# mike-gimelfarb/bboptpy

Hardware: AMD Instinct MI355X
Metric: candidate-evals/sec (higher is better)
Workload: dtype f64; 1 GPU; ActiveCMAES n=128 np=4096 rosenbrock, 256 independent populations per GPU in lockstep; populations_per_gpu=256, n=128, np=4096, objective=rosenbrock

## Files before the change

bboptpy_amd/csrc/bbo_cma.hip:

```cpp
#include "bbo_cma_kernels.hpp"
#include "bbo_sep_kernels.hpp"
#include "bbo_chol_kernels.hpp"
#include "bbo_eig_mw.hpp"

#include <algorithm>
#include <atomic>
#include <cmath>
#include <cstdlib>
#include <limits>

namespace bbo {

namespace {

enum { K_SAMPLE = 0, K_RANK, K_WHITEN, K_GRAM, K_PATHS, K_COV, K_EIGEN, K_POST, K_STOP, K_COUNT };
static const char *const K_NAMES[K_COUNT] = { "bbo:cma_sample_eval", "bbo:cma_rank", "bbo:cma_whiten", "bbo:cma_gram", "bbo:cma_paths", "bbo:cma_cov", "bbo:cma_eigen", "bbo:cma_post", "bbo:cma_history_stop" };

int pick_maxt(int ld)
{
    const int per_wave = ((ld >> 4) + 3) / 4;
    if (per_wave <= 1) return 1;
    if (per_wave <= 2) return 2;
    if (per_wave <= 4) return 4;
    return 8;
// ... 310 lines not shown
            C_.upload(cm.data(), P * ld2);
        } else {
            B_.alloc(P * ld2);
            C_.alloc(P * ld2);
            B_.upload(eye.data(), P * ld2);
            C_.upload(eye.data(), P * ld2);
        }
        isc_.upload(eye.data(), P * ld2);
    }
    D_.upload(ones.data(), P * ld);
    keep_bc_ = dense;
    last_n_ = n;

    std::vector<double> xm(P * ld, 0.);
    for (int p = 0; p < P; p++) std::copy(guess + (size_t) p * n, guess + (size_t) (p + 1) * n,
            xm.begin() + p * ld);
    xmean_.upload(xm.data(), P * ld);

    std::vector<CmaScal> sc(P);
    for (auto &s : sc) {
        std::memset(&s, 0, sizeof(s));
        s.sigma = params_.sigma0;
        s.fbest = -std::numeric_limits<double>::infinity();
        s.fworst = std::numeric_limits<double>::infinity();
        s.hist_head = -1;
        s.basis_ok = same_shape ? 0 : 1;
    }
    scal_.upload(sc.data(), P);
    basis_maybe_stale_ = same_shape;

    if (dense) eig_work_.alloc((size_t) P * 4 * eig_slab((int) ld));

    CmaDev &d = d_;
    d = CmaDev {};
    d.X = X_.p; d.f = f_.p; d.rank = rank_.p; d.order = order_.p;
    d.xmean = xmean_.p; d.xold = xold_.p; d.pc = pc_.p; d.ps = ps_.p;
    d.C = C_.p; d.B = B_.p; d.D = D_.p; d.isc = isc_.p; d.BDp = BDp_.p; d.ISp = ISp_.p;
    d.A = chol ? A_.p : nullptr;
    d.chol_repairs = chol ? chol_repairs_.p : nullptr;
    d.S = S_.p; d.zn2 = zn2_.p; d.csep = csep_.p; d.gram_part = gram_part_.p; d.mean_part = mean_part_.p;
    d.hist_best = hist_best_.p; d.hist_kth = hist_kth_.p; d.eig_work = eig_work_.p;
    d.weights = weights_.p; d.lower = lower_.p; d.upper = upper_.p; d.aux = aux_.p;
    d.zinject = nullptr; d.zrecord = nullptr; d.scal = scal_.p;
    d.stamps = stamps_.p;
    d.mw_fail_host = mw_fail_host_;
    d.mw_fault = mw_fault_from_env();
    mw_release();

    if (obj_.is_program()) {
        prog_.bind(obj_.program, params_.device, n, P);
        std::vector<ProgPlan> plan(P);
        for (int p = 0; p < P; p++)
            plan[p] = ProgPlan { X_.p + (size_t) p * c.lambda_pad * ld, f_.p + (size_t) p * c.lambda_pad, lambda,
                    c.ld };
        prog_.upload_plan(plan);
        std::vector<double> finf((size_t) P * c.lambda_pad, std::numeric_limits<double>::infinity());
        f_.upload(finf.data(), finf.size());
    } else
        prog_.unbind();

    c.honor_stop = 0;
    inited_ = true;
    if (dense) {
        launch_post(2);
        BBO_HIP(hipGetLastError());
        BBO_HIP(hipStreamSynchronize(stream_));
    }
}

void CmaEngine::launch_post(int mode)
{
    const CmaConst &c = c_;
    if (c.ld <= 128) {
        const size_t lds = (size_t) (c.ld * (c.ld + 2) + c.ld) * sizeof(double);
        allow_lds((const void*) cma_post_mfma<1>, 140 * 1024);
        allow_lds((const void*) cma_post_mfma<4>, 140 * 1024);
        if (c.npop < 32)
            hipLaunchKernelGGL(cma_post_mfma<4>, dim3(c.npop, 4), dim3(256), lds, stream_, d_, c_,
                    mode);
        else
            hipLaunchKernelGGL(cma_post_mfma<1>, dim3(c.npop, 1), dim3(256), lds, stream_, d_, c_,
                    mode);
    } else {
        dim3 grid(c.ld / 16, c.ld / 16, c.npop);
        hipLaunchKernelGGL(cma_post, grid, dim3(256), 0, stream_, d_, c_, mode);
    }
}

SampleRoute CmaEngine::sample_route() const
{
    const CmaConst &c = c_;
    SampleRoute r {};
    r.gy = c.npop;
    r.writes_zn = c.variant != 2;
    auto is = [&r](SampleKernel k, int gx, int block, size_t lds) {
        r.k = k;
        r.gx = gx;
        r.block = block;
        r.lds = lds;
    };
    if (c.variant == 2) {
        const int per_pop = std::max(1, 4096 / c.npop);
        if (c.ld <= 256)
            is(SK_SEP_16, std::min((c.lambda_pad + 15) / 16, per_pop), 256, (size_t) 16 * c.ld * sizeof(double));
        else if (c.ld <= 2048) {
            is(SK_SEP_64_512, std::min((c.lambda_pad + 7) / 8, per_pop), 512, (size_t) 8 * c.ld * sizeof(double));
            r.full = nothing_to_guard() ? 1 : 0;
            if (r.full && sep_sum_objective(c.obj) && !(d_.dbg & DBG_SEP_ROWS_LDS))
                is(c.ld == 1024 && c.obj != OBJ_RASTRIGIN && c.obj != OBJ_DIFFPOW ? SK_SEP_SUM4 : SK_SEP_SUM,
                        std::min(c.lambda_pad / (4 * SEP_K), per_pop), 256, 0);
            else if (r.full)
                r.k = SK_SEP_64_512_LEAN;
        } else
            is(SK_SEP_64, std::min((c.lambda_pad + 3) / 4, per_pop), 256, (size_t) 4 * c.ld * sizeof(double));
    } else if (c.ld == 128 && (long) c.npop * c.lambda_pad >= sample128_min_rows_
            && (c.obj < 0 || frag_objective_ok(c.obj))) {
        r.rows_per_wg = rows_per_workgroup((long) c.npop * c.lambda_pad, 4096);
        is(c.variant == 3 && chol_tri_ ? SK_EVAL128_TRI : SK_EVAL128, (c.lambda_pad + r.rows_per_wg - 1) / r.rows_per_wg,
                512, 128 * 1024);
        r.full = nothing_to_guard() ? 1 : 0;
    } else if (c.ld == 128 && (long) c.npop * (c.lambda_pad / 16) <= sample_wide_max_tiles_)
        is(c.variant == 3 && chol_tri_ ? SK_TILE8_TRI : SK_TILE8, c.lambda_pad / 16, 512,
                (size_t) 16 * (c.ld + 2) * sizeof(double));
    else if (c.ld <= 128)
        is(c.ld <= 32 ? SK_EVAL64_1_8 : c.ld <= 64 ? SK_EVAL64_1 : SK_EVAL64_2, (c.lambda_pad + 63) / 64, 256,
                (size_t) 64 * (c.ld + 2) * sizeof(double));
    else {
        const int tiles = c.lambda_pad / 16;
        const size_t lds = (size_t) 16 * (c.ld + 2) * sizeof(double);
        if ((long) tiles * c.npop <= 32 && c.ld <= 256 && !(d_.dbg & DBG_SAMPLE_4WAVES))
            is(SK_TILE16, tiles, 1024, lds);
        else
            is(pick_maxt(c.ld) == 4 ? SK_EVAL_4 : SK_EVAL_8, tiles, 256, lds);
    }
    return r;
}

void CmaEngine::launch_sample_eval()
{
    const SampleRoute r = sample_route();
    auto go = [&](auto kernel, int allow, auto... args) {
        if (allow) allow_lds((const void*) kernel, allow);
        hipLaunchKernelGGL(kernel, dim3(r.gx, r.gy), dim3(r.block), r.lds, stream_, d_, c_, args...);
    };
    timer_.begin(stream_, K_SAMPLE);
    switch (r.k) {
    case SK_NONE: break;
    case SK_SEP_16: go(sep_sample_eval<16>, 128 * 1024); break;
    case SK_SEP_64_512: go(sep_sample_eval<64, 512>, 140 * 1024); break;
    case SK_SEP_64_512_LEAN: go(sep_sample_eval<64, 512, true>, 140 * 1024); break;
    case SK_SEP_SUM: go(sep_sum_kernel<0>(c_.obj), 0); break;
    case SK_SEP_SUM4: go(sep_sum_kernel<4>(c_.obj), 0); break;
    case SK_SEP_64: go(sep_sample_eval<64>, 140 * 1024); break;
    case SK_EVAL128: go(cma_sample_eval128, 128 * 1024, r.rows_per_wg, r.full); break;
    case SK_EVAL128_TRI: go(cma_sample_eval128_tri, 128 * 1024, r.rows_per_wg, r.full); break;
    case SK_TILE8: go(cma_sample_eval<1, 8>, 0); break;
    case SK_TILE8_TRI: go(cma_sample_eval<1, 8, true>, 0); break;
    case SK_EVAL64_1_8: go(cma_sample_eval64<1, 8>, 0); break;
    case SK_EVAL64_1: go(cma_sample_eval64<1>, 80 * 1024); break;
    case SK_EVAL64_2: go(cma_sample_eval64<2>, 80 * 1024); break;
    case SK_TILE16: go(cma_sample_eval<1, 16>, 0); break;
    case SK_EVAL_4: go(cma_sample_eval<4>, 0); break;
    case SK_EVAL_8: go(cma_sample_eval<8>, 80 * 1024); break;
    }
    timer_.end(stream_);
    BBO_HIP(hipGetLastError());
    c_.use_zn = (r.writes_zn && !c_.bound) ? 1 : 0;
    last_sample_ = r;
}

void CmaEngine::launch_rank()
{
    const CmaConst &c = c_;
    rank_wrote_norms_ = false;
    timer_.begin(stream_, K_RANK);
    last_rank_ = rank_route(c.lambda, c.npop, d_.dbg);
    switch (last_rank_) {
    case RK_WAVE:
        hipLaunchKernelGGL(cma_rank_wave, dim3((c.npop + 3) / 4), dim3(256), 0, stream_, d_, c_);
        break;
    case RK_COUNT64:
        hipLaunchKernelGGL(cma_rank64, dim3((c.lambda + 3) / 4, c.npop), dim3(256), 0, stream_, d_, c_);
        break;
    case RK_COUNT32:
        hipLaunchKernelGGL(cma_rank32, dim3((c.lambda + 7) / 8, c.npop), dim3(256), 0, stream_, d_, c_);
        break;
    case RK_COUNT8:
        hipLaunchKernelGGL(cma_rank, dim3((c.lambda + 31) / 32, c.npop), dim3(256), 0, stream_, d_, c_);
        break;
    default: {
        const int m = rank_sort_m(c.lambda);
        allow_lds((const void*) cma_rank_sort, 128 * 1024);
        const size_t lds = rank_sort_merges(m, d_.dbg) ? (size_t) m * 24 : (size_t) std::max(m, 1024) * 12;
        hipLaunchKernelGGL(cma_rank_sort, dim3(c.npop), dim3(sort_threads(m)), lds, stream_, d_,
                c_, m);
        break;
    }
    }
    if (last_rank_ != RK_WAVE) rank_wrote_norms_ = c.variant == 1 && c.use_zn && !basis_maybe_stale_;
    timer_.end(stream_);
    BBO_HIP(hipGetLastError());
}

UpdateRoute CmaEngine::update_route(bool norms_done, bool with_cov) const
{
    const CmaConst &c = c_;
    UpdateRoute r {};
    auto add = [&r](UpdateKernel k, int slot, int gx, int gy, int gz, int block, size_t lds = 0, int arg = 0) {
        r.step[r.count++] = UpdateRoute::Step { k, slot, gx, gy, gz, block, lds, arg };
    };
    const int NT = c.ld / 16, LT = NT * (NT + 1) / 2;
    if (c.variant == 3) {
        const int in_lds = c.ld <= 128 ? 1 : 0;
        add(UK_CHOL_PATHS, K_PATHS, c.npop, 1, 1, 256);
        add(UK_CHOL_CPRIME, K_GRAM, LT, c.npop, 1, 256);
        add(UK_CHOL_FACTOR, K_COV, c.npop, 1, 1, 256, in_lds ? (size_t) c.ld * (c.ld + 1) * sizeof(double) : 0, in_lds);
        return r;
    }
    if (c.variant == 2) {
        add(UK_SEP_MOMENTS, K_GRAM, c.splits, (c.ld + 511) / 512, c.npop, 256);
        add(UK_SEP_PATHS, K_PATHS, c.npop, 1, 1, 256);
        return r;
    }
    if (c.variant == 1 && !norms_done) {
        if (c.ld == 128 && (long) c.npop * c.mu_pad >= 256 * 128) {
            const int rw = rows_per_workgroup((long) c.npop * c.mu_pad, 2048);
            add(UK_WHITEN128, K_WHITEN, (c.mu_pad + rw - 1) / rw, c.npop, 1, 512, (size_t) (128 * 128 + 128) * sizeof(double),
                    rw);
        } else
            add(UK_WHITEN, K_WHITEN, c.mu_pad / 16, c.npop, 1, 256, (size_t) (16 * (c.ld + 2) + 64) * sizeof(double),
                    pick_maxt(c.ld));
    }
    if (c.ld != 128)
        add(UK_GRAM, K_GRAM, c.splits, (LT + 4 * GRAM_TPW - 1) / (4 * GRAM_TPW), c.npop, 256, gram_lds_bytes(c.ld, c.rps),
                gram_ldy(c.ld));
    else if (d_.dbg & DBG_GRAM128_LDS)
        add(UK_GRAM128, K_GRAM, c.splits, c.npop, 1, 256, (size_t) (2 * G128_CH * G128_LDY + 4 * G128_CH) * sizeof(double));
    else
        add(UK_GRAM128S, K_GRAM, c.splits, c.npop, 1, 256);
    if (c.lazy_isc && c.n >= 64 && !(d_.dbg & DBG_PATHS_LAZY256))
        add(UK_PATHS_LAZY1K, K_PATHS, c.npop, 1, 1, 1024);
    else
        add(c.lazy_isc ? UK_PATHS_LAZY : UK_PATHS, K_PATHS, c.npop, 1, 1, 256);
    if (with_cov) add(UK_COV, K_COV, (c.n * (c.n + 1) / 2 + 255) / 256, c.npop, 1, 256);
    return r;
}

static auto whiten_kernel(int maxt) -> void (*)(CmaDev, CmaConst)
{
    switch (maxt) {
    case 1: return cma_whiten<1>;
    case 2: return cma_whiten<2>;
    case 4: return cma_whiten<4>;
    default: return cma_whiten<8>;
    }
}

void CmaEngine::launch_update(bool with_cov)
{
    const bool norms_done = rank_wrote_norms_;
    rank_wrote_norms_ = false;
    const UpdateRoute r = update_route(norms_done, with_cov);
    for (int i = 0; i < r.count; i++) {
        const UpdateRoute::Step &s = r.step[i];
        auto go = [&](auto kernel, int allow, auto... args) {
            if (allow) allow_lds((const void*) kernel, allow);
            hipLaunchKernelGGL(kernel, dim3(s.gx, s.gy, s.gz), dim3(s.block), s.lds, stream_, d_, c_, args...);
        };
        timer_.begin(stream_, s.slot);
        switch (s.k) {
        case UK_CHOL_PATHS: go(chol_paths, 0); break;
        case UK_CHOL_CPRIME: go(chol_cprime, 0); break;
        case UK_CHOL_FACTOR: go(chol_factor, 0, s.arg); break;
        case UK_SEP_MOMENTS: go(sep_moments, 0); break;
        case UK_SEP_PATHS: go(sep_paths, 0); break;
        case UK_WHITEN128: go(cma_whiten128, 132 * 1024, s.arg); break;
        case UK_WHITEN: go(whiten_kernel(s.arg), s.arg == 8 ? 80 * 1024 : 0); break;
        case UK_GRAM128S: go(cma_gram128s, 0); break;
        case UK_GRAM128: go(cma_gram128, 80 * 1024); break;
        case UK_GRAM: go(cma_gram, (int) GRAM_LDS_MAX, s.arg); break;
        case UK_PATHS: go(cma_paths, 0); break;
        case UK_PATHS_LAZY: go(cma_paths_lazy, 0); break;
        case UK_PATHS_LAZY1K: go(cma_paths_lazy1k, 0); break;
        case UK_COV: go(cma_cov, 0); break;
        }
        timer_.end(stream_);
        BBO_HIP(hipGetLastError());
    }
    last_update_ = r;
}

int CmaEngine::next_mw_xcd()
{
    static std::atomic<int> counter { 0 };
    return counter.fetch_add(1) & 7;
}

EigRoute CmaEngine::eig_route(bool spread_ok, bool fuse_ok) const
{
    const CmaConst &c = c_;
    const int dbg = d_.dbg;
    EigRoute r {};
    if (c.variant >= 2) return r;
    auto add = [&r](EigKernel k, int arg = 0) { r.step[r.count++] = EigRoute::Step { k, arg }; };
    const EigPlan pl_lds = eig_plan(c.n, c.ld);
    r.split = pl_lds.use_lds && pl_lds.threads == 512 && pl_lds.dc && c.npop <= split_maxp_
            && !(dbg & (DBG_QL | DBG_DC_NO_MERGES | DBG_DC_NO_LEAVES | DBG_TRED_L2 | DBG_EIG_ONE_WG));
    const EigPlan pl = r.split ? eig_plan_split(c.n, c.ld) : pl_lds;
// ... 259 lines not shown
        launch_eigen(eig_route());
        BBO_HIP(hipStreamSynchronize(stream_));
    }
    timer_.collect();
    prog_timer_.collect();
}

void CmaEngine::inject_normals(const double *z, int count)
{
    BBO_REQUIRE(inited_, "inject_normals before init");
    rank_wrote_norms_ = false;
    if (!z) {
        d_.zinject = nullptr;
        return;
    }
    const size_t want = (size_t) c_.npop * c_.lambda * c_.n;
    BBO_REQUIRE((size_t) count == want, "inject_normals: count must be populations*lambda*n");
    if (zinject_.count != want) zinject_.alloc(want);
    zinject_.upload(z, want);
    d_.zinject = zinject_.p;
}

void CmaEngine::after_chunk(bool in_run)
{
    if (in_run) return;
    if (mw_check_failed()) {
        launch_eigen(eig_route());
        BBO_HIP(hipStreamSynchronize(stream_));
    }
}

void CmaEngine::inspect(const std::vector<CmaScal> &sc)
{
    bool stale = false;
    for (const auto &s : sc) stale = stale || !s.basis_ok;
    basis_maybe_stale_ = stale;
    mw_check_failed();
    for (const auto &s : sc)
        if (s.eig_mw_fail && !mw_disabled_) {
            mw_disabled_ = true;
            mw_release();
        }
}

int CmaEngine::chunk_limit(int want)
{
    return small_fused_ok() ? std::min(want, 512) : want;
}

void CmaEngine::launch_chunk(int gens)
{
    if (small_fused_ok()) launch_small(gens, true);
    else Engine::launch_chunk(gens);
}

void CmaEngine::solution(int population, double *x_out, int *n_evals, int *converged)
{
    enter_population("solution()", population);
    CmaScal s;
    scal_.download(&s, 1, population);
    std::vector<double> x(c_.ld);
    if (s.it <= 0) xmean_.download(x.data(), c_.ld, (size_t) population * c_.ld);
    else X_.download(x.data(), c_.ld, ((size_t) population * c_.lambda_pad + s.ibw[0]) * c_.ld);
    std::copy(x.begin(), x.begin() + c_.n, x_out);
    *n_evals = s.fev;
    if (s.it <= 0) {
        *converged = c_.variant == 3 ? (c_.tol >= 0. ? 1 : 0) : (0 >= c_.mit) ? 1 : 0;
    } else {
        *converged = s.flag != 0 ? 1 : 0;
    }
}

void CmaEngine::optimize(int n, const double *lower, const double *upper, const double *guess,
        const ObjectiveSpec &obj, double *x_out, int *n_evals, int *converged)
{
    init(n, lower, upper, guess, obj);
    const int max_gen = c_.mfev / c_.lambda + 2;
    run(max_gen);
    CmaScal s;
    scal_.download(&s, 1, 0);
    std::vector<double> x(c_.ld);
    if (s.it <= 0) xmean_.download(x.data(), c_.ld, 0);
    else X_.download(x.data(), c_.ld, (size_t) s.ibw[0] * c_.ld);
    std::copy(x.begin(), x.begin() + c_.n, x_out);
    *n_evals = s.fev;
    *converged = (s.stop == 1) ? 1 : 0;
}

double CmaEngine::evaluate_point(const double *x)
{
    if (obj_.needs_host()) {
        double f = 0.;
        obj_.eval_host(x, 1, c_.n, c_.n, &f);
        return f;
    }
    if (obj_.is_program()) {
        BBO_HIP(hipSetDevice(params_.device));
        return prog_.evaluate_point(stream_, x);
    }
    return builtin_objective_host(obj_.builtin, c_.n, x, aux_h_.data());
}

int CmaEngine::get(const std::string &k, int p, double *out, int cap)
{
    enter_population("get()", p);
    const CmaConst &c = c_;
    const size_t ld = c.ld, n = c.n;
    const StateOut o { out, cap };
    if (c.variant == 2 && (k == "B" || k == "C" || k == "invsqrtC" || k == "ycoeff"))
        throw Error(BBO_ERR_KEY, "SepCMAES keeps a diagonal covariance: read 'csep' and 'D'");
    if (c.variant == 3 && (k == "B" || k == "C" || k == "D" || k == "invsqrtC" || k == "ycoeff" || k == "csep"))
        throw Error(BBO_ERR_KEY, "CholeskyCMAES keeps the factor: read 'A'");
    if (k == "A") {
        if (c.variant != 3) throw Error(BBO_ERR_KEY, "'A' belongs to CholeskyCMAES");
        return o.rows(A_, p * ld, c.n, c.n, c.ld);
    }
    if (k == "xmean") return o.vec(xmean_, p * ld, (int) n);
    if (k == "xold") return o.vec(xold_, p * ld, (int) n);
    if (k == "pc") return o.vec(pc_, p * ld, (int) n);
    if (k == "ps") return o.vec(ps_, p * ld, (int) n);
    if (k == "D") return o.vec(D_, p * ld, (int) n);
    if (k == "csep") return o.vec(csep_, p * ld, (int) n);
    if (k == "B") return o.rows(B_, p * ld, c.n, c.n, c.ld);
    if (k == "C") return o.rows(C_, p * ld, c.n, c.n, c.ld);
    if (k == "invsqrtC") {
        if (c.lazy_isc && out) {
            const int hs = c_.honor_stop;
            c_.honor_stop = 0;
            launch_post(3);
            c_.honor_stop = hs;
            BBO_HIP(hipGetLastError());
            BBO_HIP(hipStreamSynchronize(stream_));
        }
        return o.rows(isc_, p * ld, c.n, c.n, c.ld);
    }
    if (k == "BD") {
        if (out && cap >= (int) (n * n)) {
            std::vector<double> pk(ld * ld);
            BDp_.download(pk.data(), ld * ld, p * ld * ld);
            for (size_t i = 0; i < n; i++)
                for (size_t j = 0; j < n; j++) out[i * n + j] = pk[bfrag_index(i, j, ld)];
        }
        return (int) (n * n);
    }
    if (k == "arx") return o.rows(X_, (size_t) p * c.lambda_pad, c.lambda, c.n, c.ld);
    if (k == "weights") {
        if (out && cap >= c.mu) weights_.download(out, c.mu);
        return c.mu;
    }
    if (k == "fitness") {
        if (out && cap >= c.lambda) f_.download(out, c.lambda, (size_t) p * c.lambda_pad);
        return c.lambda;
    }
    if (k == "fit_idx" || k == "fit_val" || k == "rank") {
        if (out && cap >= c.lambda) {
            std::vector<int> ord(c.lambda);
            (k == "rank" ? rank_ : order_).download(ord.data(), c.lambda,
                    (size_t) p * c.lambda_pad);
            if (k == "fit_val") {
                std::vector<double> f(c.lambda);
                f_.download(f.data(), c.lambda, (size_t) p * c.lambda_pad);
                for (int i = 0; i < c.lambda; i++) out[i] = f[ord[i]];
            } else {
                for (int i = 0; i < c.lambda; i++) out[i] = ord[i];
            }
        }
        return c.lambda;
    }
    if (k == "ycoeff") {
        if (out && cap >= c.mu) {
            std::vector<double> S(c.mu_pad);
            S_.download(S.data(), c.mu_pad, (size_t) p * c.mu_pad);
            for (int i = 0; i < c.mu; i++) out[i] = S[i] / std::max(S[c.mu - 1 - i], 1e-8);
        }
        return c.mu;
    }
    if (k == "zlast") {
        const size_t cnt = (size_t) c.lambda * n;
        if (!zrecord_.p) return 0;
        if (out && cap >= (int) cnt) zrecord_.download(out, cnt, p * cnt);
        return (int) cnt;
    }
    if (k == "profile") return profile_report(out, cap);
    if (const int r = prog_get(k, out, cap); r >= 0) return r;
    if (k == "eig_work") {
        const size_t cnt = std::min((size_t) 4 * eig_slab(c.ld), eig_work_.count);
        if (out && (size_t) cap >= cnt) eig_work_.download(out, cnt, (size_t) p * 4 * eig_slab(c.ld));
        return (int) cnt;
    }
    if (k == "eig_stamps") {
        if (!stamps_.p) return 0;
        if (out && cap >= 48) {
            long long t[48];
            stamps_.download(t, 48);
            for (int i = 0; i < 48; i++) out[i] = (double) t[i];
        }
        return 48;
    }
    if (k == "best_hist" || k == "kth_hist") {
        if (out && cap >= c.hlen)
            (k == "best_hist" ? hist_best_ : hist_kth_).download(out, c.hlen, (size_t) p * c.hlen);
        return c.hlen;
    }
    CmaScal s;
    scal_.download(&s, 1, p);
    if (k == "sigma") return o.one(s.sigma);
    if (k == "it") return o.one(s.it);
    if (k == "fev") return o.one(s.fev);
    if (k == "flag") return o.one(s.flag);
    if (k == "stop") return o.one(s.stop);
    if (k == "hsig") return o.one(s.hsig);
    if (k == "pslen") return o.one(s.pslen);
    if (k == "fbest") return o.one(s.fbest);
    if (k == "fworst") return o.one(s.fworst);
    if (k == "eigenlastev") return o.one(s.eigenlastev);
    if (k == "eigen_done") return o.one(s.eigen_done);
    if (k == "basis_ok") return o.one(s.basis_ok);
    if (k == "eig_stage") return o.one(s.eig_stage);
    if (k == "eig_mw_fail") return o.one(s.eig_mw_fail);
    if (k == "chol_repairs") {
        if (c.variant != 3) throw Error(BBO_ERR_KEY, "'chol_repairs' belongs to CholeskyCMAES");
        int r = 0;
        chol_repairs_.download(&r, 1, p);
        return o.one(r);
    }
    if (c.variant == 3 && k == "chol_tri") return o.one(chol_tri_ ? 1 : 0);
    if (c.variant == 3 && k == "stol") return o.one(c.stol);
    if (c.variant == 3 && k == "ranked") return o.one(c.ranked);
    if (k == "eig_mw_off") return o.one(mw_disabled_ ? 1 : 0);
    if (k == "eig_split_maxp") return o.one(split_maxp_);
    if (k == "eig_fixed128") return o.one(last_route_.fixed ? 1 : 0);
    if (k == "cov_fused") return o.one(last_route_.forms_c ? 1 : 0);
    if (k == "eig_route") {
        double ids[sizeof(last_route_.step) / sizeof(last_route_.step[0])];
        for (int i = 0; i < last_route_.count; i++) ids[i] = last_route_.step[i].k;
        return o.copy(ids, last_route_.count);
    }
    if (k == "rank_route") return o.one(last_rank_);
    if (k == "sample_route") return o.one(last_sample_.k);
    if (k == "sample_lean") return o.one(last_sample_.full);
    if (k == "update_route") {
        double ids[sizeof(last_update_.step) / sizeof(last_update_.step[0])];
        for (int i = 0; i < last_update_.count; i++) ids[i] = last_update_.step[i].k;
        return o.copy(ids, last_update_.count);
    }
    if (k == "small_fused") return o.one(small_fused_ ? 1 : 0);
    if (k == "splits") return o.one(c.splits);
    if (k == "eig_mw_reserved") return o.one((double) mw_reserved_);
    if (k == "eig_mw_capacity") {
        MwBudget &b = MwBudget::get();
        std::lock_guard<std::mutex> lock(b.m);
        return o.one((double) b.capacity(params_.device));
    }
    if (k == "best_len") return o.one(s.hist_len);
    if (k == "best_buffer") return o.one(s.hist_head);
    if (k == "ibest") return o.one(s.ibw[0]);
    if (k == "ybw") return o.copy(s.ybw, 4);
    if (k == "ibw") {
        const double ids[4] = { (double) s.ibw[0], (double) s.ibw[1], (double) s.ibw[2], (double) s.ibw[3] };
        return o.copy(ids, 4);
    }
    if (k == "n") return o.one(c.n);
    if (k == "lambda") return o.one(c.lambda);
    if (k == "mu") return o.one(c.mu);
    if (k == "mueff") return o.one(c.mueff);
    if (k == "cc") return o.one(c.cc);
    if (k == "cs") return o.one(c.cs);
    if (k == "c1") return o.one(c.c1);
    if (k == "cmu") return o.one(c.cmu);
    if (k == "cneg") return o.one(c.cneg);
    if (k == "alphaold") return o.one(c.alphaold);
    if (k == "cm") return o.one(c.cm);
    if (k == "ccov") return o.one(c.ccov);
    if (k == "damps") return o.one(c.damps);
    if (k == "chi") return o.one(c.chi);
    if (k == "eigenfreq") return o.one(c.eigenfreq);
    if (k == "hlen") return o.one(c.hlen);
    if (k == "ik") return o.one(c.ik);
    if (k == "mit") return o.one(c.mit);
    if (k == "mfev") return o.one(c.mfev);
    if (k == "sigma0") return o.one(c.sigma0);
    throw Error(BBO_ERR_KEY, "unknown state key '" + k + "'");
}

int CmaEngine::set(const std::string &k, int p, const double *in, int count)
{
    enter_population("set()", p);
    rank_wrote_norms_ = false;
    const CmaConst &c = c_;
    const size_t ld = c.ld, n = c.n;
    auto vec_in = [&](DevBuf<double> &b) {
        BBO_REQUIRE(count == (int) n, "set: wrong element count");
        upload_rows(b, p, 1, c.n, c.ld, in);
        return count;
    };
    auto mat_in = [&](DevBuf<double> &b) {
        BBO_REQUIRE(count == (int) (n * n), "set: wrong element count");
        std::vector<double> tmp(ld * ld, 0.);
        for (size_t i = 0; i < n; i++) std::copy(in + i * n, in + (i + 1) * n, tmp.begin() + i * ld);
        b.upload(tmp.data(), ld * ld, p * ld * ld);
        return count;
    };
    if (c.variant == 2 && (k == "B" || k == "C" || k == "D"))
        throw Error(BBO_ERR_KEY, "SepCMAES: set 'csep' (D is its square root)");
    if (c.variant == 3 && (k == "B" || k == "C" || k == "D" || k == "csep"))
        throw Error(BBO_ERR_KEY, "CholeskyCMAES keeps the factor: set 'A'");
// ... 147 lines not shown
```

bboptpy_amd/csrc/bbo_cma_kernels.hpp:

```cpp
#pragma once

#include "bbo_cma.hpp"
#include "bbo_objectives.hpp"
#include "bbo_rng.hpp"
#include "bbo_eig.hpp"
#include "bbo_rank.hpp"

namespace bbo {

typedef double d4_t __attribute__((ext_vector_type(4)));

#define BBO_INF (__builtin_huge_val())

__device__ inline void cma_draw_quad(const CmaDev &d, const CmaConst &c, int p, int row, int q,
        int gen, uint32_t sw, const double2 *tab, double (&z)[4])
{
    const int j0 = cma_quad_col0(q);
    z[0] = z[1] = z[2] = z[3] = 0.;
    if (row < c.lambda && j0 < c.n) {
        if (d.zinject) {
            const double *zi = d.zinject + ((size_t) p * c.lambda + row) * c.n;
#pragma unroll
            for (int i = 0; i < 4; i++)
                if (j0 + 4 * i < c.n) z[i] = zi[j0 + 4 * i];
        } else {
            normal_quad(c.seed, (uint32_t) row, (uint32_t) q, (uint32_t) gen, sw, tab, z[0], z[1],
                    z[2], z[3]);
#pragma unroll
            for (int i = 1; i < 4; i++)
                if (j0 + 4 * i >= c.n) z[i] = 0.;
        }
        if (d.zrecord) {
            double *zr = d.zrecord + ((size_t) p * c.lambda + row) * c.n;
#pragma unroll
            for (int i = 0; i < 4; i++)
                if (j0 + 4 * i < c.n) zr[j0 + 4 * i] = z[i];
        }
    }
}

__device__ inline uint32_t cma_draw_quad_fast(const CmaDev &d, const CmaConst &c, int p, int row,
        int q, int gen, uint32_t sw, const double2 *tab, double (&z)[4])
{
    const int j0 = cma_quad_col0(q);
    uint32_t pend = 0;
    z[0] = z[1] = z[2] = z[3] = 0.;
    if (row < c.lambda && j0 < c.n) {
        if (d.zinject) {
            const double *zi = d.zinject + ((size_t) p * c.lambda + row) * c.n;
#pragma unroll
            for (int i = 0; i < 4; i++)
                if (j0 + 4 * i < c.n) z[i] = zi[j0 + 4 * i];
        } else {
            pend = normal_quad_fast(c.seed, (uint32_t) row, (uint32_t) q, (uint32_t) gen, sw, tab,
                    z[0], z[1], z[2], z[3]);
#pragma unroll
            for (int i = 1; i < 4; i++)
                if (j0 + 4 * i >= c.n) {
                    z[i] = 0.;
                    pend &= ~(1u << i);
                }
        }
        if (d.zrecord) {
            double *zr = d.zrecord + ((size_t) p * c.lambda + row) * c.n;
#pragma unroll
            for (int i = 0; i < 4; i++)
                if (j0 + 4 * i < c.n) zr[j0 + 4 * i] = z[i];
        }
    }
    return pend;
}

__device__ inline double cma_settle_draw(const CmaDev &d, const CmaConst &c, int p, int row, int q,
        int slot, int gen, uint32_t sw, const double2 *tab)
{
    const double v = normal_quad_settle(c.seed, (uint32_t) row, (uint32_t) q, (uint32_t) slot,
            (uint32_t) gen, sw, tab, zig_global_f());
    if (d.zrecord)
        d.zrecord[((size_t) p * c.lambda + row) * c.n + cma_quad_col0(q) + 4 * slot] = v;
    return v;
}

template<int MAXT, int NW = 4, bool TRI = false>
__global__ __launch_bounds__(64 * NW) void cma_sample_eval(CmaDev d, CmaConst c)
{
    const int p = blockIdx.y, mt = blockIdx.x;
    const CmaScal *sc = d.scal + p;
    if (pop_frozen(c, sc)) return;
    extern __shared__ double lds[];
    const int tid = threadIdx.x, lane = tid & 63, wave = tid >> 6;
    const int ld = c.ld, ldz = ld + 2;
    const int gen = sc->it;

    __shared__ double2 ntab[NORMAL_TABLE_N];
    normal_table_fill(ntab, tid, 64 * NW);
    __syncthreads();
    const int nquads = ld >> 2;
    const uint32_t sw = stream_word(STREAM_CMA_NORMAL, (uint32_t) p);
    uint64_t pend = 0;
    for (int qi = tid, it = 0; qi < 16 * nquads; qi += 64 * NW, it++) {
        const int r = qi / nquads, q = qi - r * nquads;
        double z[4];
        pend |= (uint64_t) cma_draw_quad_fast(d, c, p, mt * 16 + r, q, gen, sw, ntab, z) << (4 * it);
        const int j0 = cma_quad_col0(q);
#pragma unroll
        for (int i = 0; i < 4; i++) lds[r * ldz + j0 + 4 * i] = z[i];
    }
    while (pend) {
        const int b = __ffsll((unsigned long long) pend) - 1;
        pend &= pend - 1;
        const int qi = tid + 64 * NW * (b >> 2), r = qi / nquads, q = qi - r * nquads;
        lds[r * ldz + cma_quad_col0(q) + 4 * (b & 3)] =
                cma_settle_draw(d, c, p, mt * 16 + r, q, b & 3, gen, sw, ntab);
    }
    __syncthreads();

    d4_t acc[MAXT];
#pragma unroll
    for (int t = 0; t < MAXT; t++) acc[t] = d4_t { 0., 0., 0., 0. };
    const int NT = ld >> 4, KS = ld >> 2;
    const double *bdp = d.BDp + (size_t) p * ld * ld;
    const int ar = lane & 15, ak = lane >> 4;
    double zz = 0.;
    for (int ks0 = 0; ks0 < KS; ks0 += 4) {
        double a[4], b[4][MAXT];
#pragma unroll
        for (int u = 0; u < 4; u++) {
            a[u] = lds[ar * ldz + 4 * (ks0 + u) + ak];
#pragma unroll
            for (int t = 0; t < MAXT; t++) {
                const int nt = wave + NW * t;
                b[u][t] = (nt < NT && (!TRI || ks0 + u < 4 * (nt + 1)))
                        ? bdp[((size_t) nt * KS + ks0 + u) * 64 + lane] : 0.;
            }
        }
#pragma unroll
        for (int u = 0; u < 4; u++) {
            zz = __builtin_fma(a[u], a[u], zz);
#pragma unroll
            for (int t = 0; t < MAXT; t++) {
                const int nt = wave + NW * t;
                if (nt < NT && (!TRI || ks0 + u < 4 * (nt + 1)))
                    acc[t] = __builtin_amdgcn_mfma_f64_16x16x4f64(a[u], b[u][t], acc[t], 0, 0, 0);
            }
        }
    }
    zz += __shfl_xor(zz, 16, 64);
    zz += __shfl_xor(zz, 32, 64);
    if (wave == 0 && ak == 0) d.zn2[(size_t) p * c.lambda_pad + mt * 16 + ar] = zz;
    __syncthreads();

    const double sigma = sc->sigma;
    const double *xm = d.xmean + (size_t) p * ld;
    double *Xp = d.X + (size_t) p * c.lambda_pad * ld;
    double xmc[MAXT], loc[MAXT], upc[MAXT];
#pragma unroll
    for (int t = 0; t < MAXT; t++) {
        const int col = min((wave + NW * t) * 16 + (lane & 15), ld - 1);
        xmc[t] = xm[col];
        loc[t] = c.bound ? d.lower[col] : 0.;
        upc[t] = c.bound ? d.upper[col] : 0.;
    }
#pragma unroll
// ... 5 lines not shown
            for (int r = 0; r < 4; r++) {
                const int rl = (lane >> 4) + 4 * r;
                double v = 0.;
                if (col < c.n) {
                    v = xmc[t] + sigma * acc[t][r];
                    if (c.bound) v = fmax(loc[t], fmin(v, upc[t]));
                }
                lds[rl * ldz + col] = v;
                Xp[((size_t) mt * 16 + rl) * ld + col] = v;
            }
        }
    }
    __syncthreads();

    if (c.obj >= 0 && tid < 256) {
        const int r = tid >> 4, g = tid & 15;
        double f = eval_row_group<16>(c.obj, c.n, &lds[r * ldz], d.aux, g);
        if (g == 0) {
            const int row = mt * 16 + r;
            if (!(row < c.lambda) || f != f) f = BBO_INF;
            d.f[(size_t) p * c.lambda_pad + row] = f;
        }
    }
}

template<int MAXT, int KSM = 32>
__device__ __forceinline__ void sample_eval64_body(const CmaDev &d, const CmaConst &c, int p, int bx,
        double *lds, int psub,
        bool stage_table = true)
{
    const int row0 = bx * 64;
    const CmaScal *sc = d.scal + p;
    if (pop_frozen(c, sc)) return;
    const int tid = threadIdx.x, lane = tid & 63, wave = tid >> 6;
    const int ld = c.ld, ldz = ld + 2;
    const int gen = sc->it;
    const int NT = ld >> 4, KS = ld >> 2;

    const double *bdp = d.BDp + (size_t) p * ld * ld;
    double bfr[MAXT][KSM];
#pragma unroll
    for (int t = 0; t < MAXT; t++) {
        const int nt = wave + 4 * t;
#pragma unroll
        for (int ks = 0; ks < KSM; ks++)
            bfr[t][ks] = (nt < NT && ks < KS) ? bdp[((size_t) nt * KS + ks) * 64 + lane] : 0.;
    }

    __shared__ double2 ntab[NORMAL_TABLE_N];
    if (stage_table) {
        normal_table_fill(ntab, tid, 256);
        __syncthreads();
    }
    const int nquads = ld >> 2;
    const uint32_t sw = stream_word(STREAM_CMA_NORMAL, (uint32_t) psub);
    uint32_t pend = 0;
    for (int qi = tid, it = 0; qi < 64 * nquads; qi += 256, it++) {
        const int r = qi / nquads, q = qi - r * nquads;
        double z[4];
        pend |= cma_draw_quad_fast(d, c, p, row0 + r, q, gen, sw, ntab, z) << (4 * it);
        const int j0 = cma_quad_col0(q);
#pragma unroll
        for (int i = 0; i < 4; i++) lds[r * ldz + j0 + 4 * i] = z[i];
    }
    while (pend) {
        const int b = __ffs(pend) - 1;
        pend &= pend - 1;
        const int qi = tid + 256 * (b >> 2), r = qi / nquads, q = qi - r * nquads;
        lds[r * ldz + cma_quad_col0(q) + 4 * (b & 3)] =
                cma_settle_draw(d, c, p, row0 + r, q, b & 3, gen, sw, ntab);
    }
    __syncthreads();

    d4_t acc[4][MAXT];
    const int ar = lane & 15, ak = lane >> 4;
#pragma unroll
    for (int mt = 0; mt < 4; mt++) {
        double zz = 0.;
#pragma unroll
        for (int t = 0; t < MAXT; t++) acc[mt][t] = d4_t { 0., 0., 0., 0. };
#pragma unroll
        for (int ks = 0; ks < KSM; ks++) {
            if (ks < KS) {
                const double a = lds[(mt * 16 + ar) * ldz + 4 * ks + ak];
                zz = __builtin_fma(a, a, zz);
#pragma unroll
                for (int t = 0; t < MAXT; t++)
                    acc[mt][t] = __builtin_amdgcn_mfma_f64_16x16x4f64(a, bfr[t][ks], acc[mt][t], 0, 0, 0);
            }
        }
        zz += __shfl_xor(zz, 16, 64);
        zz += __shfl_xor(zz, 32, 64);
        if (wave == 0 && ak == 0 && row0 + mt * 16 + ar < c.lambda_pad)
            d.zn2[(size_t) p * c.lambda_pad + row0 + mt * 16 + ar] = zz;
    }
    __syncthreads();

    const double sigma = sc->sigma;
    const double *xm = d.xmean + (size_t) p * ld;
    double *Xp = d.X + (size_t) p * c.lambda_pad * ld;
    double xmc[MAXT], loc[MAXT], upc[MAXT];
#pragma unroll
    for (int t = 0; t < MAXT; t++) {
        const int col = min((wave + 4 * t) * 16 + (lane & 15), ld - 1);
        xmc[t] = xm[col];
        loc[t] = c.bound ? d.lower[col] : 0.;
        upc[t] = c.bound ? d.upper[col] : 0.;
    }
#pragma unroll
    for (int mt = 0; mt < 4; mt++) {
#pragma unroll
        for (int t = 0; t < MAXT; t++) {
            const int nt = wave + 4 * t;
            if (nt < NT) {
                const int col = nt * 16 + (lane & 15);
#pragma unroll
                for (int r = 0; r < 4; r++) {
                    const int rl = mt * 16 + (lane >> 4) + 4 * r;
                    double v = 0.;
                    if (col < c.n) {
                        v = xmc[t] + sigma * acc[mt][t][r];
                        if (c.bound) v = fmax(loc[t], fmin(v, upc[t]));
                    }
                    lds[rl * ldz + col] = v;
                    if (row0 + rl < c.lambda_pad) Xp[((size_t) row0 + rl) * ld + col] = v;
                }
            }
        }
    }
    __syncthreads();

    if (c.obj >= 0) {
        const int g = tid & 15;
#pragma unroll
        for (int rr = 0; rr < 4; rr++) {
            const int r = (tid >> 4) + 16 * rr;
            double f = eval_row_group<16>(c.obj, c.n, &lds[r * ldz], d.aux, g);
            const int row = row0 + r;
            if (g == 0 && row < c.lambda_pad) {
                if (!(row < c.lambda) || f != f) f = BBO_INF;
                d.f[(size_t) p * c.lambda_pad + row] = f;
            }
        }
    }
}

template<int MAXT, int KSM = 32>
__global__ __launch_bounds__(256) void cma_sample_eval64(CmaDev d, CmaConst c)
{
    extern __shared__ __attribute__((aligned(16))) double lds[];
    sample_eval64_body<MAXT, KSM>(d, c, blockIdx.y, blockIdx.x, lds, blockIdx.y);
}

template<bool FULL>
__device__ inline void sample128_epilogue(const CmaDev &d, const CmaConst &c, int p, int rowbase,
        double sigma, const d4_t (&acc)[8], int lane, const double *xm)
{
    const int fr = lane & 15, fk = lane >> 4;
    const int n = FULL ? 128 : c.n;
    double *Xp = d.X + (size_t) p * c.lambda_pad * 128 + ((size_t) rowbase + fk) * 128 + fr;
    double x[8][4];
#pragma unroll
    for (int t = 0; t < 8; t++) {
        const int col = t * 16 + fr;
        const double xmc = xm[col];
#pragma unroll
        for (int r = 0; r < 4; r++) {
            double v = 0.;
            if (FULL) {
                v = xmc + sigma * acc[t][r];
            } else if (col < n) {
                v = xmc + sigma * acc[t][r];
                if (c.bound) v = fmax(d.lower[col], fmin(v, d.upper[col]));
            }
            x[t][r] = v;
            Xp[(size_t) (4 * r) * 128 + t * 16] = v;
        }
    }
    if (c.obj >= 0) {
        double f[4];
        eval_frag_rows<8>(c.obj, n, x, d.aux, lane, f);
        if (fr == 0) {
#pragma unroll
            for (int r = 0; r < 4; r++) {
                const int rr = rowbase + fk + 4 * r;
                double fv = f[r];
                if ((!FULL && !(rr < c.lambda)) || fv != fv) fv = BBO_INF;
                d.f[(size_t) p * c.lambda_pad + rr] = fv;
            }
        }
    }
}

template<bool FULL, bool TRI = false>
__device__ __forceinline__ void sample_eval128_body(const CmaDev &d, const CmaConst &c,
        int rows_per_wg, double *bd, const double2 *ntab, const double *ftab, const double *xms)
{
    const int p = blockIdx.y, row0 = blockIdx.x * rows_per_wg;
    const CmaScal *sc = d.scal + p;
    const int tid = threadIdx.x, lane = tid & 63, wave = tid >> 6;
    const int gen = sc->it;
    const double sigma = sc->sigma;
    const int tiles = min(rows_per_wg, c.lambda_pad - row0) >> 4;
    const int fr = lane & 15, fk = lane >> 4;
    const uint32_t sw = stream_word(STREAM_CMA_NORMAL, (uint32_t) p);

    for (int tile = wave; tile < tiles; tile += 8) {
        const int rowbase = row0 + tile * 16;
        const int row = rowbase + fr;
        d4_t acc[8];
#pragma unroll
        for (int t = 0; t < 8; t++) acc[t] = d4_t { 0., 0., 0., 0. };
        double zz = 0.;
        if (FULL) {
            double z[32];
            uint32_t pend = normal_quads_fast<8>(c.seed, (uint32_t) row, (uint32_t) fk, 4u,
                    (uint32_t) gen, sw, ntab, z);
            while (pend) {
                const int b = __ffs(pend) - 1;
                pend &= pend - 1;
                const double v = normal_quad_settle(c.seed, (uint32_t) row,
                        (uint32_t) (4 * (b >> 2) + fk), (uint32_t) (b & 3), (uint32_t) gen, sw,
                        ntab, ftab);
#pragma unroll
                for (int i = 0; i < 32; i++) z[i] = (i == b) ? v : z[i];
            }
#pragma unroll
            for (int i = 0; i < 32; i++) zz = __builtin_fma(z[i], z[i], zz);
            int hi = lane + 8192;
            asm volatile("" : "+v"(hi));
            auto frag = [&](int i, int t) {
                const int idx = (i >> 3) * 8 + t * 32 + (i & 7);
                return idx < 128 ? bd[lane + idx * 64] : bd[hi + (idx - 128) * 64];
            };
            double pre[8];
#pragma unroll
            for (int t = 0; t < 8; t++) pre[t] = frag(0, t);
#pragma unroll
            for (int i = 0; i < 32; i++) {
#pragma unroll
                for (int t = 0; t < 8; t++) {
                    if (TRI && (i >> 2) > t) continue;
                    const double bv = (i & 3) == 0 ? pre[t] : frag(i, t);
                    acc[t] = __builtin_amdgcn_mfma_f64_16x16x4f64(z[i], bv, acc[t], 0, 0, 0);
                }
                if ((i & 3) == 3) {
                    if (i + 1 < 32) {
#pragma unroll
                        for (int t = 0; t < 8; t++)
                            if (!TRI || ((i + 1) >> 2) <= t) pre[t] = frag(i + 1, t);
                    }
                    __builtin_amdgcn_sched_barrier(0);
                }
            }
        } else {
#pragma unroll 1
            for (int kc = 0; kc < 4; kc++) {
                double a[8];
#pragma unroll
                for (int h = 0; h < 2; h++) {
                    double z[4];
                    cma_draw_quad(d, c, p, row, 4 * (2 * kc + h) + fk, gen, sw, ntab, z);
#pragma unroll
                    for (int i = 0; i < 4; i++) {
                        a[4 * h + i] = z[i];
                        zz = __builtin_fma(z[i], z[i], zz);
                    }
                }
                const double *bk = bd + kc * 8 * 64 + lane;
#pragma unroll
                for (int i = 0; i < 8; i++) {
#pragma unroll
                    for (int t = 0; t < 8; t++) {
                        if (TRI && 2 * kc + (i >> 2) > t) continue;
                        acc[t] = __builtin_amdgcn_mfma_f64_16x16x4f64(a[i], bk[(t * 32 + i) * 64],
                                acc[t], 0, 0, 0);
                    }
                }
            }
        }
        zz += __shfl_xor(zz, 16, 64);
        zz += __shfl_xor(zz, 32, 64);
        if (fk == 0) d.zn2[(size_t) p * c.lambda_pad + row] = zz;
        sample128_epilogue<FULL>(d, c, p, rowbase, sigma, acc, lane, xms);
    }
}

__global__ __launch_bounds__(512, 1) void cma_sample_eval128(CmaDev d, CmaConst c, int rows_per_wg,
        int full)
{
    const int p = blockIdx.y;
    const CmaScal *sc = d.scal + p;
    if (pop_frozen(c, sc)) return;
    extern __shared__ __attribute__((aligned(16))) double bd[];
    const int tid = threadIdx.x;
    {
        const double2 *src = reinterpret_cast<const double2*>(d.BDp + (size_t) p * 128 * 128);
        double2 *dst = reinterpret_cast<double2*>(bd);
#pragma unroll
        for (int i = 0; i < 16; i++) dst[tid + 512 * i] = src[tid + 512 * i];
    }
    __shared__ double2 ntab[NORMAL_TABLE_N];
    __shared__ double ftab[NORMAL_FTABLE_N];
    __shared__ double xms[128];
    normal_table_fill(ntab, tid, 512);
    normal_ftable_fill(ftab, tid, 512);
    if (tid < 128) xms[tid] = d.xmean[(size_t) p * 128 + tid];
    __syncthreads();
    if (full) sample_eval128_body<true>(d, c, rows_per_wg, bd, ntab, ftab, xms);
    else sample_eval128_body<false>(d, c, rows_per_wg, bd, ntab, ftab, xms);
}

__global__ __launch_bounds__(512, 1) void cma_sample_eval128_tri(CmaDev d, CmaConst c, int rows_per_wg,
        int full)
{
    const int p = blockIdx.y;
    const CmaScal *sc = d.scal + p;
    if (pop_frozen(c, sc)) return;
    extern __shared__ __attribute__((aligned(16))) double bd[];
    const int tid = threadIdx.x;
    {
        const double2 *src = reinterpret_cast<const double2*>(d.BDp + (size_t) p * 128 * 128);
        double2 *dst = reinterpret_cast<double2*>(bd);
#pragma unroll
        for (int i = 0; i < 16; i++) dst[tid + 512 * i] = src[tid + 512 * i];
    }
    __shared__ double2 ntab[NORMAL_TABLE_N];
    __shared__ double ftab[NORMAL_FTABLE_N];
    __shared__ double xms[128];
    normal_table_fill(ntab, tid, 512);
    normal_ftable_fill(ftab, tid, 512);
    if (tid < 128) xms[tid] = d.xmean[(size_t) p * 128 + tid];
    __syncthreads();
    if (full) sample_eval128_body<true, true>(d, c, rows_per_wg, bd, ntab, ftab, xms);
    else sample_eval128_body<false, true>(d, c, rows_per_wg, bd, ntab, ftab, xms);
}

template<int SL>
__device__ __forceinline__ void cma_rank_body(const CmaDev &d, const CmaConst &c)
{
    const int p = blockIdx.y;
    CmaScal *sc = d.scal + p;
    if (pop_frozen(c, sc)) return;
    __shared__ __attribute__((aligned(16))) double tile[RANK_TILE];
    const int tid = threadIdx.x;
    const int cand = blockIdx.x * (256 / SL) + tid / SL, slice = tid % SL;
    const double *f = d.f + (size_t) p * c.lambda_pad;
    const bool live = cand < c.lambda;
    const int cnt = rank_by_counting<SL>(f, c.lambda, cand, slice, tile);
    const bool norms = c.variant == 1 && c.use_zn && sc->basis_ok;
    if (live && slice == 0) {
        const double fi = f[cand];
        d.rank[(size_t) p * c.lambda_pad + cand] = cnt;
        d.order[(size_t) p * c.lambda_pad + cnt] = cand;
        if (cnt == 0) { sc->ibw[0] = cand; sc->ybw[0] = fi; }
        if (cnt == 1) { sc->ibw[1] = cand; sc->ybw[1] = fi; }
        if (cnt == c.lambda - 2) { sc->ibw[2] = cand; sc->ybw[2] = fi; }
        if (cnt == c.lambda - 1) { sc->ibw[3] = cand; sc->ybw[3] = fi; }
        if (norms && cnt >= c.lambda - c.mu)
            d.S[(size_t) p * c.mu_pad + cnt - (c.lambda - c.mu)] =
                    sc->sigma * sc->sigma * d.zn2[(size_t) p * c.lambda_pad + cand];
    }
    if (norms && blockIdx.x == 0)
        for (int wr = c.mu + tid; wr < c.mu_pad; wr += 256) d.S[(size_t) p * c.mu_pad + wr] = 0.;
    if (blockIdx.x == 0 && tid == 0) sc->fev += c.lambda;
}

__global__ __launch_bounds__(256) void cma_rank(CmaDev d, CmaConst c)
{
    cma_rank_body<8>(d, c);
}
__global__ __launch_bounds__(256) void cma_rank32(CmaDev d, CmaConst c)
{
    cma_rank_body<32>(d, c);
}
__global__ __launch_bounds__(256) void cma_rank64(CmaDev d, CmaConst c)
{
    cma_rank_body<64>(d, c);
}

static_assert((int) DBG_RANK_COUNT32 == RANK_DBG_COUNT32 && (int) DBG_RANK_COUNT_NO64 == RANK_DBG_COUNT_NO64
        && (int) DBG_RANK_BITONIC == RANK_DBG_BITONIC, "bbo_rank.hpp reads these bits of CmaDev::dbg");

__global__ __launch_bounds__(1024) void cma_rank_sort(CmaDev d, CmaConst c, int m)
{
    const int p = blockIdx.x;
    CmaScal *sc = d.scal + p;
    if (pop_frozen(c, sc)) return;
    extern __shared__ __attribute__((aligned(16))) double sortbuf[];
    double *keys = sortbuf;
    int *idx = reinterpret_cast<int*>(sortbuf + max(m, 1024));
    const double *f = d.f + (size_t) p * c.lambda_pad;
    int *order = d.order + (size_t) p * c.lambda_pad, *rank = d.rank + (size_t) p * c.lambda_pad;
    if (rank_sort_merges(m, d.dbg)) {
        int *ibuf = reinterpret_cast<int*>(sortbuf + 2 * m);
        if (m == 2048) merge_sort_lds<2>(f, c.lambda, sortbuf, ibuf, order, rank, &keys, &idx);
        else merge_sort_lds<4>(f, c.lambda, sortbuf, ibuf, order, rank, &keys, &idx);
    } else
    bitonic_sort_lds(f, c.lambda, m, keys, idx, order, rank);
    if (c.variant == 1 && c.use_zn && sc->basis_ok) {
        const double s2 = sc->sigma * sc->sigma;
        for (int wr = threadIdx.x; wr < c.mu_pad; wr += blockDim.x)
            d.S[(size_t) p * c.mu_pad + wr] = wr < c.mu
                    ? s2 * d.zn2[(size_t) p * c.lambda_pad + idx[c.lambda - c.mu + wr]] : 0.;
    }
    if (threadIdx.x == 0) {
        const int L = c.lambda;
        sc->ibw[0] = idx[0]; sc->ybw[0] = keys[0];
        sc->ibw[1] = idx[1]; sc->ybw[1] = keys[1];
        sc->ibw[2] = idx[L - 2]; sc->ybw[2] = keys[L - 2];
        sc->ibw[3] = idx[L - 1]; sc->ybw[3] = keys[L - 1];
        sc->fev += L;
    }
}

__device__ __forceinline__ void rank_wave_body(const CmaDev &d, const CmaConst &c, int p, int lane)
{
    CmaScal *sc = d.scal + p;
    if (pop_frozen(c, sc)) return;
    const double *f = d.f + (size_t) p * c.lambda_pad;
    double kf[1] = { lane < c.lambda ? f[lane] : __builtin_huge_val() };
    int ki[1] = { lane < c.lambda ? lane : 0x7fffffff };
    for (int k = 2; k <= 64; k <<= 1)
        for (int j = k >> 1; j > 0; j >>= 1) {
            switch (j) {
            case 1: sort_wave_stage<1, 1>(kf, ki, lane, j, k); break;
            case 2: sort_wave_stage<1, 2>(kf, ki, lane, j, k); break;
            case 4: sort_wave_stage<1, 4>(kf, ki, lane, j, k); break;
            case 8: sort_wave_stage<1, 8>(kf, ki, lane, j, k); break;
            case 16: sort_wave_stage<1, 16>(kf, ki, lane, j, k); break;
            default: sort_wave_stage<1, 32>(kf, ki, lane, j, k); break;
            }
        }
    const int L = c.lambda;
    if (lane < L) {
        d.order[(size_t) p * c.lambda_pad + lane] = ki[0];
        d.rank[(size_t) p * c.lambda_pad + ki[0]] = lane;
        if (lane == 0) { sc->ibw[0] = ki[0]; sc->ybw[0] = kf[0]; }
        if (lane == 1) { sc->ibw[1] = ki[0]; sc->ybw[1] = kf[0]; }
        if (lane == L - 2) { sc->ibw[2] = ki[0]; sc->ybw[2] = kf[0]; }
        if (lane == L - 1) { sc->ibw[3] = ki[0]; sc->ybw[3] = kf[0]; }
    }
    if (lane == 0) sc->fev += L;
}

__global__ __launch_bounds__(256) void cma_rank_wave(CmaDev d, CmaConst c)
{
    const int p = blockIdx.x * 4 + (threadIdx.x >> 6), lane = threadIdx.x & 63;
    if (p >= c.npop) return;
    rank_wave_body(d, c, p, lane);
}

template<int MAXT>
__device__ __forceinline__ void whiten_body(const CmaDev &d, const CmaConst &c, int p, int mt,
        double *lds)
{
    const CmaScal *sc = d.scal + p;
    if (pop_frozen(c, sc)) return;
    const int tid = threadIdx.x, lane = tid & 63, wave = tid >> 6;
    const int ld = c.ld, ldz = ld + 2;
    if (c.use_zn && sc->basis_ok) {
        if (tid < 16) {
            const int wr = mt * 16 + tid;
            if (wr < c.mu_pad)
                d.S[(size_t) p * c.mu_pad + wr] = wr < c.mu
                        ? sc->sigma * sc->sigma * d.zn2[(size_t) p * c.lambda_pad
                                + d.order[(size_t) p * c.lambda_pad + c.lambda - c.mu + wr]]
                        : 0.;
        }
        return;
    }
    double *part = lds + 16 * ldz;
    const double *Xp = d.X + (size_t) p * c.lambda_pad * ld;
    const double *xold = d.xmean + (size_t) p * ld;
    const int *order = d.order + (size_t) p * c.lambda_pad;

    for (int q = tid; q < 16 * ld; q += 256) {
        const int r = q / ld, j = q - r * ld;
        const int wr = mt * 16 + r;
        double v = 0.;
        if (wr < c.mu && j < c.n) {
            const int cand = order[c.lambda - c.mu + wr];
            v = Xp[(size_t) cand * ld + j] - xold[j];
        }
        lds[r * ldz + j] = v;
    }
    __syncthreads();

// ... 1299 lines not shown
```

Measured before the change: 719.7 million candidate-evals/s.

## Specialize full 128-dim sample kernels with slim args and wave-uniform z patching

Splits the 128-dim sampling kernels into template-specialized variants so the FULL path is compiled as its own kernel, with a compact argument struct and compile-time constants for n, ld and lambda. It also replaces the per-lane select-into-32-registers loop for rejected normal draws with a wave-uniform scalar-index store into vector registers, aiming to avoid dynamic register indexing and scratch spills. A zn2 debug accessor is added. The cost is more kernel instantiations and more complex inline-asm-guarded code.

```diff
diff --git a/bboptpy_amd/csrc/bbo_cma.hip b/bboptpy_amd/csrc/bbo_cma.hip
--- a/bboptpy_amd/csrc/bbo_cma.hip
+++ b/bboptpy_amd/csrc/bbo_cma.hip
@@ -486,8 +486,19 @@
     case SK_SEP_SUM: go(sep_sum_kernel<0>(c_.obj), 0); break;
     case SK_SEP_SUM4: go(sep_sum_kernel<4>(c_.obj), 0); break;
     case SK_SEP_64: go(sep_sample_eval<64>, 140 * 1024); break;
-    case SK_EVAL128: go(cma_sample_eval128, 128 * 1024, r.rows_per_wg, r.full); break;
-    case SK_EVAL128_TRI: go(cma_sample_eval128_tri, 128 * 1024, r.rows_per_wg, r.full); break;
+    case SK_EVAL128:
+    case SK_EVAL128_TRI:
+        if (r.full) {
+            const Sample128Args a { d_.BDp, d_.X, d_.f, d_.zn2, d_.xmean, d_.scal, d_.aux, c_.seed, c_.lambda_pad,
+                    c_.obj, r.rows_per_wg, c_.honor_stop };
+            auto kernel = r.k == SK_EVAL128 ? cma_sample_eval128_full : cma_sample_eval128_tri_full;
+            allow_lds((const void*) kernel, 128 * 1024);
+            hipLaunchKernelGGL(kernel, dim3(r.gx, r.gy), dim3(r.block), r.lds, stream_, a);
+        } else if (r.k == SK_EVAL128)
+            go(cma_sample_eval128, 128 * 1024, r.rows_per_wg);
+        else
+            go(cma_sample_eval128_tri, 128 * 1024, r.rows_per_wg);
+        break;
     case SK_TILE8: go(cma_sample_eval<1, 8>, 0); break;
     case SK_TILE8_TRI: go(cma_sample_eval<1, 8, true>, 0); break;
     case SK_EVAL64_1_8: go(cma_sample_eval64<1, 8>, 0); break;
@@ -1053,6 +1064,10 @@
         if (out && cap >= c.lambda) f_.download(out, c.lambda, (size_t) p * c.lambda_pad);
         return c.lambda;
     }
+    if (k == "zn2") {
+        if (out && cap >= c.lambda) zn2_.download(out, c.lambda, (size_t) p * c.lambda_pad);
+        return c.lambda;
+    }
     if (k == "fit_idx" || k == "fit_val" || k == "rank") {
         if (out && cap >= c.lambda) {
             std::vector<int> ord(c.lambda);
diff --git a/bboptpy_amd/csrc/bbo_cma_kernels.hpp b/bboptpy_amd/csrc/bbo_cma_kernels.hpp
--- a/bboptpy_amd/csrc/bbo_cma_kernels.hpp
+++ b/bboptpy_amd/csrc/bbo_cma_kernels.hpp
@@ -9,6 +9,7 @@
 namespace bbo {
 
 typedef double d4_t __attribute__((ext_vector_type(4)));
+typedef double d16_t __attribute__((ext_vector_type(16)));
 
 #define BBO_INF (__builtin_huge_val())
 
@@ -320,6 +321,29 @@
     sample_eval64_body<MAXT, KSM>(d, c, blockIdx.y, blockIdx.x, lds, blockIdx.y);
 }
 
+__device__ __forceinline__ void store_by_wave_index(d16_t &zlo, d16_t &zhi, int b, double v)
+{
+    unsigned long long todo = __builtin_amdgcn_ballot_w64(true);
+    while (todo) {
+        const int s = __builtin_amdgcn_readlane(b, __builtin_ctzll(todo));
+        int u = s;
+        asm("" : "+s"(u));
+        const bool mine = b == s;
+        todo &= ~__builtin_amdgcn_ballot_w64(mine);
+        if (mine) {
+            asm volatile("");
+            if (u < 16) {
+                asm volatile("");
+                zlo[u & 15] = v;
+            }
+            if (u >= 16) {
+                asm volatile("");
+                zhi[u & 15] = v;
+            }
+        }
+    }
+}
+
 template<bool FULL>
 __device__ inline void sample128_epilogue(const CmaDev &d, const CmaConst &c, int p, int rowbase,
         double sigma, const d4_t (&acc)[8], int lane, const double *xm)
@@ -384,14 +408,24 @@
             double z[32];
             uint32_t pend = normal_quads_fast<8>(c.seed, (uint32_t) row, (uint32_t) fk, 4u,
                     (uint32_t) gen, sw, ntab, z);
+            d16_t zlo, zhi;
+#pragma unroll
+            for (int i = 0; i < 16; i++) {
+                zlo[i] = z[i];
+                zhi[i] = z[16 + i];
+            }
             while (pend) {
                 const int b = __ffs(pend) - 1;
                 pend &= pend - 1;
                 const double v = normal_quad_settle(c.seed, (uint32_t) row,
                         (uint32_t) (4 * (b >> 2) + fk), (uint32_t) (b & 3), (uint32_t) gen, sw,
                         ntab, ftab);
-#pragma unroll
-                for (int i = 0; i < 32; i++) z[i] = (i == b) ? v : z[i];
+                store_by_wave_index(zlo, zhi, b, v);
+            }
+#pragma unroll
+            for (int i = 0; i < 16; i++) {
+                z[i] = zlo[i];
+                z[16 + i] = zhi[i];
             }
 #pragma unroll
             for (int i = 0; i < 32; i++) zz = __builtin_fma(z[i], z[i], zz);
@@ -454,8 +488,8 @@
     }
 }
 
-__global__ __launch_bounds__(512, 1) void cma_sample_eval128(CmaDev d, CmaConst c, int rows_per_wg,
-        int full)
+template<bool FULL, bool TRI>
+__device__ __forceinline__ void sample_eval128_kernel(const CmaDev &d, const CmaConst &c, int rows_per_wg)
 {
     const int p = blockIdx.y;
     const CmaScal *sc = d.scal + p;
@@ -475,33 +509,54 @@
     normal_ftable_fill(ftab, tid, 512);
     if (tid < 128) xms[tid] = d.xmean[(size_t) p * 128 + tid];
     __syncthreads();
-    if (full) sample_eval128_body<true>(d, c, rows_per_wg, bd, ntab, ftab, xms);
-    else sample_eval128_body<false>(d, c, rows_per_wg, bd, ntab, ftab, xms);
-}
-
-__global__ __launch_bounds__(512, 1) void cma_sample_eval128_tri(CmaDev d, CmaConst c, int rows_per_wg,
-        int full)
-{
-    const int p = blockIdx.y;
-    const CmaScal *sc = d.scal + p;
-    if (pop_frozen(c, sc)) return;
-    extern __shared__ __attribute__((aligned(16))) double bd[];
-    const int tid = threadIdx.x;
-    {
-        const double2 *src = reinterpret_cast<const double2*>(d.BDp + (size_t) p * 128 * 128);
-        double2 *dst = reinterpret_cast<double2*>(bd);
-#pragma unroll
-        for (int i = 0; i < 16; i++) dst[tid + 512 * i] = src[tid + 512 * i];
-    }
-    __shared__ double2 ntab[NORMAL_TABLE_N];
-    __shared__ double ftab[NORMAL_FTABLE_N];
-    __shared__ double xms[128];
-    normal_table_fill(ntab, tid, 512);
-    normal_ftable_fill(ftab, tid, 512);
-    if (tid < 128) xms[tid] = d.xmean[(size_t) p * 128 + tid];
-    __syncthreads();
-    if (full) sample_eval128_body<true, true>(d, c, rows_per_wg, bd, ntab, ftab, xms);
-    else sample_eval128_body<false, true>(d, c, rows_per_wg, bd, ntab, ftab, xms);
+    sample_eval128_body<FULL, TRI>(d, c, rows_per_wg, bd, ntab, ftab, xms);
+}
+
+__global__ __launch_bounds__(512, 1) void cma_sample_eval128(CmaDev d, CmaConst c, int rows_per_wg)
+{
+    sample_eval128_kernel<false, false>(d, c, rows_per_wg);
+}
+
+__global__ __launch_bounds__(512, 1) void cma_sample_eval128_tri(CmaDev d, CmaConst c, int rows_per_wg)
+{
+    sample_eval128_kernel<false, true>(d, c, rows_per_wg);
+}
+
+struct Sample128Args {
+    const double *BDp;
+    double *X, *f, *zn2;
+    const double *xmean;
+    CmaScal *scal;
+    const double *aux;
+    uint64_t seed;
+    int lambda_pad, obj, rows_per_wg, honor_stop;
+};
+template<bool TRI>
+__device__ __forceinline__ void sample_eval128_full(const Sample128Args &a)
+{
+    CmaDev d {};
+    d.BDp = const_cast<double*>(a.BDp);
+    d.X = a.X;
+    d.f = a.f;
+    d.zn2 = a.zn2;
+    d.xmean = const_cast<double*>(a.xmean);
+    d.scal = a.scal;
+    d.aux = a.aux;
+    CmaConst c {};
+    c.n = c.ld = 128;
+    c.lambda = c.lambda_pad = a.lambda_pad;
+    c.obj = a.obj;
+    c.seed = a.seed;
+    c.honor_stop = a.honor_stop;
+    sample_eval128_kernel<true, TRI>(d, c, a.rows_per_wg);
+}
+__global__ __launch_bounds__(512, 1) void cma_sample_eval128_full(Sample128Args a)
+{
+    sample_eval128_full<false>(a);
+}
+__global__ __launch_bounds__(512, 1) void cma_sample_eval128_tri_full(Sample128Args a)
+{
+    sample_eval128_full<true>(a);
 }
 
 template<int SL>
```

Measured after the change: 721.3 million candidate-evals/s (median of 6 runs). About the same (+0.2%).
